# microsoft/ANCE

Measured on NVIDIA H100. Metric: ANN-refresh throughput: passages encoded/sec + queries top-200/sec, 8.8M x 768, higher is better.
Workload: dtype fp16

## Files before the change

ance_b200/csrc/attention.cuh:

```cuda
#pragma once
#include "act16.cuh"
#include "tc05.cuh"

namespace attn {

using namespace tc05;

constexpr int kTile = 128;
constexpr int kDh = 64;

__device__ __forceinline__ float ex2_ftz(float x) {
  float r;
  asm("ex2.approx.ftz.f32 %0, %1;" : "=f"(r) : "f"(x));
  return r;
}

struct Params {
  int n_tokens;
  int L;
  int heads;
  int hidden;
  const float* kbias;
  float scale_log2;
  const int32_t* row_lo;
  const int32_t* row_hi;
  const int2* tile_kv;
};

struct Smem {
  static constexpr int kStages = 3;
  static constexpr int kTileBytes = kTile * kDh * 2;
  static constexpr int kQ = 0;
  static constexpr int kKV = kQ + kTileBytes;
  static constexpr int kP = kKV + kStages * 2 * kTileBytes;
  static constexpr int kSPitch = kTile + 4;
  static constexpr int kS = kP + kTile * kTile * 2;
  static constexpr int kBias = kS + kTile * kSPitch * 4;
  static constexpr int kBiasStride = kTile * 4 + 16;
  static constexpr int kBar = kBias + kBiasStride;
  static constexpr int kNumBars = 2 + 2 * kStages;
  static constexpr int kTotal = kBar + kNumBars * 8;
  static constexpr int kDynamic = kTotal + 1024;
  static_assert(kDynamic <= 232448, "attention smem exceeds 227 KB");
};

constexpr float kRealMax = -7000.0f;

constexpr int kThreads = 256;

template <bool kPacked, bool kSingle, uint32_t FMT>
__global__ void __launch_bounds__(kThreads, 1)
attention_kernel(const __grid_constant__ CUtensorMap tmQKV, const __grid_constant__ CUtensorMap tmCTX, const Params p) {
  extern __shared__ uint8_t smem_raw[];
  uint8_t* smem = reinterpret_cast<uint8_t*>((reinterpret_cast<uintptr_t>(smem_raw) + 1023) & ~uintptr_t(1023));
  uint64_t* bars = reinterpret_cast<uint64_t*>(smem + Smem::kBar);
  uint64_t* q_full = bars + 0;
  uint64_t* q_empty = bars + 1;
  uint64_t* kv_full = bars + 2;
  uint64_t* kv_empty = bars + 2 + Smem::kStages;

  const int warp = threadIdx.x >> 5, lane = threadIdx.x & 31;
  const int n_tiles = (p.n_tokens + kTile - 1) / kTile;
  const int total_work = n_tiles * p.heads;
  const int nkv_dense = (p.L >= kTile) ? p.L / kTile : 1;
  auto kv_of = [&](int tile, int& kv0, int& nkv) {
    if constexpr (kPacked && !kSingle) {
      const int2 t = __ldg(p.tile_kv + tile);
      kv0 = t.x;
      nkv = t.y;
    } else {
      kv0 = (p.L >= kTile) ? (tile * kTile / p.L) * p.L : tile * kTile;
      nkv = nkv_dense;
    }
  };

  if (warp == 0 && lane == 0) {
    tma_prefetch_desc(&tmQKV);
    tma_prefetch_desc(&tmCTX);
    mbar_init(q_full, 1);
    mbar_init(q_empty, 4);
    for (int s = 0; s < Smem::kStages; ++s) {
      mbar_init(&kv_full[s], 1);
      mbar_init(&kv_empty[s], 4);
    }
    fence_barrier_init();
  }
  __syncthreads();

  if (warp == 0) {
    if (lane == 0) {
      Ring<Smem::kStages> kv;
      uint32_t qc = 0;
      for (int w = blockIdx.x; w < total_work; w += gridDim.x) {
        const int tile = w / p.heads, h = w - tile * p.heads;
        const int tok0 = tile * kTile;
        int kv_tok0, nkv;
        kv_of(tile, kv_tok0, nkv);
        for (int j = 0; j < nkv; ++j) {
          if (j == 0) {
            mbar_wait(q_empty, (qc & 1) ^ 1, 10);
            ++qc;
            mbar_arrive_expect_tx(q_full, Smem::kTileBytes);
            tma_load_2d(smem + Smem::kQ, &tmQKV, q_full, h * kDh, tok0, kEvictFirst);
          }
          mbar_wait(&kv_empty[kv.stage], kv.phase ^ 1, 11);
          mbar_arrive_expect_tx(&kv_full[kv.stage], 2 * Smem::kTileBytes);
          uint8_t* st = smem + Smem::kKV + kv.stage * 2 * Smem::kTileBytes;
          tma_load_2d(st, &tmQKV, &kv_full[kv.stage], p.hidden + h * kDh, kv_tok0 + j * kTile, kEvictNormal);
          tma_load_2d(st + Smem::kTileBytes, &tmQKV, &kv_full[kv.stage], 2 * p.hidden + h * kDh, kv_tok0 + j * kTile,
                      kEvictNormal);
          kv.advance();
        }
      }
    }
  } else if (warp >= 4) {
    const int quad = warp & 3;
    const int row = quad * 32 + lane;
    uint8_t* sP = smem + Smem::kP;
    float* sS = reinterpret_cast<float*>(smem + Smem::kS);
    const uint32_t srow = smem_u32(sS) / 4u + static_cast<uint32_t>(row * Smem::kSPitch);
    float* sbias = reinterpret_cast<float*>(smem + Smem::kBias);
    unsigned* smask = reinterpret_cast<unsigned*>(sbias + kTile);
    const int bar_id = 1;
    const uint32_t sq = smem_u32(smem + Smem::kQ);
    const uint32_t sp = smem_u32(sP);
    Ring<Smem::kStages> kv;
    uint32_t qc = 0;
    auto load_bias = [&](int w2, int j2) -> float {
      if (w2 >= total_work) return 0.f;
      int k0, nk;
      kv_of(w2 / p.heads, k0, nk);
      const int kt = k0 + j2 * kTile + row;
      return (kt < p.n_tokens) ? __ldg(p.kbias + kt) : -INFINITY;
    };
    auto store_chunks = [&](uint8_t* rowp, int chunk0, const uint32_t* pk) {
#pragma unroll
      for (int q = 0; q < 4; ++q) {
        const int ch = (chunk0 + q) ^ (row & 7);
        *reinterpret_cast<uint4*>(rowp + ch * 16) = make_uint4(pk[q * 4], pk[q * 4 + 1], pk[q * 4 + 2], pk[q * 4 + 3]);
      }
    };
    float bv = load_bias(blockIdx.x, 0);
    for (int w = blockIdx.x; w < total_work; w += gridDim.x) {
      const int tile = w / p.heads, h = w - tile * p.heads;
      const int tok0 = tile * kTile;
      int kv0, nkv;
      kv_of(tile, kv0, nkv);
      const bool varlen = kPacked && p.row_lo != nullptr;
      int seq_lo = (p.L >= kTile) ? 0 : (row / p.L) * p.L;
      int seq_hi = (p.L >= kTile) ? kTile : seq_lo + p.L;
      if (varlen) {
        seq_lo = __ldg(p.row_lo + tok0 + row) - kv0;
        seq_hi = __ldg(p.row_hi + tok0 + row) - kv0;
      }
      const int seq_full = seq_lo + ((seq_hi - seq_lo) & ~31);
      float m_run = -INFINITY, l_run = 0.f;
      float o[kDh];
      if constexpr (!kSingle) {
#pragma unroll
        for (int i = 0; i < kDh; ++i) o[i] = 0.f;
      }
      for (int j = 0; j < nkv; ++j) {
        sbias[row] = bv;
        {
          const unsigned mk = __ballot_sync(0xffffffffu, bv < 0.f);
          if (lane == 0) smask[quad] = mk;
        }
        if (row == 0) bulk_wait_read_all();
        named_bar_sync(bar_id, kTile);
        bv = (j + 1 < nkv) ? load_bias(w, j + 1) : load_bias(w + gridDim.x, 0);
        const unsigned mk[4] = {smask[0], smask[1], smask[2], smask[3]};
        const int bl = seq_lo - j * kTile, bh = seq_hi - j * kTile;
        const int bf = seq_full - j * kTile;
        const bool plain = kPacked ? (varlen && bl <= 0 && bh >= kTile) : ((mk[0] | mk[1] | mk[2] | mk[3]) == 0u);
        int st[4];
        if (varlen) {
#pragma unroll
          for (int c = 0; c < 4; ++c)
            st[c] = (bh <= c * 32 || bl >= c * 32 + 32) ? 0 : (bl <= c * 32 && (kSingle ? bh : bf) >= c * 32 + 32) ? 1 : 2;
        } else {
          bool own[4], any_unmasked = false;
#pragma unroll
          for (int c = 0; c < 4; ++c) {
            own[c] = !kPacked || (p.L >= 32 ? (c * 32 >= seq_lo && c * 32 < seq_hi) : c == quad);
            any_unmasked |= own[c] && mk[c] != 0xffffffffu;
          }
          const bool skip_ok = (kPacked && p.L < 32) ? false : (any_unmasked || (!kSingle && m_run > kRealMax));
#pragma unroll
          for (int c = 0; c < 4; ++c)
            st[c] = !own[c] ? 0 : (mk[c] == 0xffffffffu && skip_ok) ? 0 : (mk[c] == 0u && !(kPacked && p.L < 32)) ? 1 : 2;
        }
        if (j == 0) mbar_wait(q_full, qc & 1, 12);
        mbar_wait(&kv_full[kv.stage], kv.phase, 13);
        const uint32_t sk = smem_u32(smem + Smem::kKV + kv.stage * 2 * Smem::kTileBytes);
        {
          float s0[kTile / 2], s1[kTile / 2];
#pragma unroll
          for (int i = 0; i < kTile / 2; ++i) s0[i] = s1[i] = 0.f;
          wgmma_fence();
#pragma unroll
          for (int k = 0; k < kDh / 16; ++k) {
            const uint64_t bdesc = make_desc_k_sw128(sk + k * 32);
            wgmma_n128<FMT, 0>(s0, make_desc_k_sw128(sq + k * 32), bdesc, 1u);
            wgmma_n128<FMT, 0>(s1, make_desc_k_sw128(sq + 64 * 128 + k * 32), bdesc, 1u);
          }
          wgmma_commit();
          wgmma_wait<0>();
          wgmma_fence_regs(s0);
          wgmma_fence_regs(s1);
          acc_store_frag(sS, Smem::kSPitch, 0, 0, s0);
          acc_store_frag(sS, Smem::kSPitch, 64, 0, s1);
        }
        if (j == nkv - 1) {
          __syncwarp();
          if (lane == 0) mbar_arrive(q_empty);
          ++qc;
        }
        named_bar_sync(bar_id, kTile);
        float rsum, alpha = 1.f, m_new;
        bool all_skip = false;
        if constexpr (kSingle) {
          uint32_t v[kTile];
#pragma unroll
          for (int c = 0; c < kTile; c += 32) acc_ld_x32(srow + c, v + c);
          float mx[4] = {-INFINITY, -INFINITY, -INFINITY, -INFINITY};
          if (plain) {
#pragma unroll
            for (int i = 0; i < kTile; ++i) mx[i & 3] = fmaxf(mx[i & 3], __uint_as_float(v[i]));
          } else {
#pragma unroll
            for (int c = 0; c < kTile; c += 32) {
              if (st[c >> 5] == 1) {
#pragma unroll
                for (int i = c; i < c + 32; ++i) {
                  const float t = __uint_as_float(v[i]) * p.scale_log2;
                  v[i] = __float_as_uint(t);
                  mx[i & 3] = fmaxf(mx[i & 3], t);
                }
              } else if (st[c >> 5] == 2) {
#pragma unroll
                for (int i = c; i < c + 32; ++i) {
                  float t = fmaf(__uint_as_float(v[i]), p.scale_log2, sbias[i]);
                  if (kPacked && (i < bl || i >= bh)) t = -INFINITY;
                  v[i] = __float_as_uint(t);
                  mx[i & 3] = fmaxf(mx[i & 3], t);
                }
              }
            }
          }
          m_new = fmaxf(fmaxf(mx[0], mx[1]), fmaxf(mx[2], mx[3]));
          const float sc = plain ? p.scale_log2 : 1.0f;
          if (plain) m_new *= p.scale_log2;
          const float nm = -m_new;
          float rs[4] = {0.f, 0.f, 0.f, 0.f};
#pragma unroll
          for (int c = 0; c < kTile; c += 32) {
            uint32_t pk[16];
            if (st[c >> 5] == 0) {
#pragma unroll
              for (int i = 0; i < 16; ++i) pk[i] = 0u;
            } else {
#pragma unroll
              for (int i = 0; i < 32; i += 2) {
                const float p0 = ex2_ftz(fmaf(__uint_as_float(v[c + i]), sc, nm));
                const float p1 = ex2_ftz(fmaf(__uint_as_float(v[c + i + 1]), sc, nm));
                rs[(i >> 1) & 3] += p0 + p1;
                pk[i >> 1] = act16::Act<FMT>::pack2(p0, p1);
              }
            }
            store_chunks(sP + (c >> 6) * (kTile * 128) + row * 128, (c & 63) >> 3, pk);
          }
          rsum = (rs[0] + rs[1]) + (rs[2] + rs[3]);
        } else {
          const int stb = st[0] | (st[1] << 2) | (st[2] << 4) | (st[3] << 6);
          all_skip = stb == 0;
          auto exp_pass = [&](float m_ref, float& rs_out) -> float {
            float rs_ = 0.f, mu = -INFINITY;
            const float nm = -m_ref;
#pragma unroll 1
            for (int c = 0; c < kTile; c += 32) {
              const int sc_ = (stb >> (c >> 4)) & 3;
              uint32_t pk[16];
              if (sc_ == 0) {
#pragma unroll
                for (int i = 0; i < 16; ++i) pk[i] = 0u;
              } else {
                uint32_t v[32];
                acc_ld_x32(srow + c, v);
                if (sc_ == 1) {
#pragma unroll
                  for (int i = 0; i < 32; i += 2) {
                    const float u0 = fmaf(__uint_as_float(v[i]), p.scale_log2, nm);
                    const float u1 = fmaf(__uint_as_float(v[i + 1]), p.scale_log2, nm);
                    mu = fmaxf(mu, fmaxf(u0, u1));
                    const float p0 = ex2_ftz(u0), p1 = ex2_ftz(u1);
                    rs_ += p0 + p1;
                    pk[i >> 1] = act16::Act<FMT>::pack2(p0, p1);
                  }
                } else {
#pragma unroll
                  for (int i = 0; i < 32; i += 2) {
                    float u0 = fmaf(__uint_as_float(v[i]), p.scale_log2, sbias[c + i]) + nm;
                    float u1 = fmaf(__uint_as_float(v[i + 1]), p.scale_log2, sbias[c + i + 1]) + nm;
                    if constexpr (kPacked) {
                      const int k0 = c + i, k1 = c + i + 1;
                      u0 = (k0 < bl || k0 >= bh) ? -INFINITY : (k0 < bf) ? fmaf(__uint_as_float(v[i]), p.scale_log2, nm) : u0;
                      u1 = (k1 < bl || k1 >= bh) ? -INFINITY : (k1 < bf) ? fmaf(__uint_as_float(v[i + 1]), p.scale_log2, nm) : u1;
                    }
                    mu = fmaxf(mu, fmaxf(u0, u1));
                    const float p0 = ex2_ftz(u0), p1 = ex2_ftz(u1);
                    rs_ += p0 + p1;
                    pk[i >> 1] = act16::Act<FMT>::pack2(p0, p1);
                  }
                }
              }
              store_chunks(sP + (c >> 6) * (kTile * 128) + row * 128, (c & 63) >> 3, pk);
            }
            rs_out = rs_;
            return mu;
          };
          const bool optimistic = __all_sync(0xffffffffu, j > 0 && m_run > kRealMax);
          if (optimistic) {
            m_new = m_run;
            alpha = 1.f;
            rsum = 0.f;
            float over = -INFINITY;
            if (!all_skip) {
              over = exp_pass(m_run, rsum);
            } else {
              float dummy;
              exp_pass(m_run, dummy);
            }
            if (__any_sync(0xffffffffu, over > 8.0f)) {
              m_new = fmaxf(m_run, m_run + over);
              alpha = exp2f(m_run - m_new);
              exp_pass(m_new, rsum);
            }
          } else {
            float m_blk = -INFINITY;
            if (!all_skip) {
#pragma unroll 1
              for (int c = 0; c < kTile; c += 32) {
                const int sc_ = (stb >> (c >> 4)) & 3;
                if (sc_ == 0) continue;
                uint32_t v[32];
                acc_ld_x32(srow + c, v);
                if (plain) {
#pragma unroll
                  for (int i = 0; i < 32; ++i) m_blk = fmaxf(m_blk, __uint_as_float(v[i]));
                } else if (sc_ == 1) {
#pragma unroll
                  for (int i = 0; i < 32; ++i) m_blk = fmaxf(m_blk, __uint_as_float(v[i]) * p.scale_log2);
                } else {
#pragma unroll
                  for (int i = 0; i < 32; ++i) {
                    float t = fmaf(__uint_as_float(v[i]), p.scale_log2, sbias[c + i]);
                    if (kPacked && (c + i < bl || c + i >= bh)) t = -INFINITY;
                    m_blk = fmaxf(m_blk, t);
                  }
                }
              }
            }
            if (plain) m_blk *= p.scale_log2;
            m_new = fmaxf(m_run, m_blk);
            alpha = (m_run == -INFINITY) ? 0.f : exp2f(m_run - m_new);
            exp_pass(m_new, rsum);
          }
        }
        fence_proxy_async_smem();
        named_bar_sync(bar_id, kTile);
        {
          const uint32_t sv = sk + Smem::kTileBytes;
          float o0[kDh / 2], o1[kDh / 2];
#pragma unroll
          for (int i = 0; i < kDh / 2; ++i) o0[i] = o1[i] = 0.f;
          wgmma_fence();
#pragma unroll
          for (int k = 0; k < kTile / 16; ++k) {
            const uint32_t pa = sp + (k >> 2) * (kTile * 128) + (k & 3) * 32;
            const uint64_t bdesc = make_desc_mn_sw128(sv + k * 2048, kTile * 128, 1024);
            wgmma_n64<FMT, 1>(o0, make_desc_k_sw128(pa), bdesc, 1u);
            wgmma_n64<FMT, 1>(o1, make_desc_k_sw128(pa + 64 * 128), bdesc, 1u);
          }
          wgmma_commit();
          wgmma_wait<0>();
          wgmma_fence_regs(o0);
          wgmma_fence_regs(o1);
          __syncwarp();
          if (lane == 0) mbar_arrive(&kv_empty[kv.stage]);
          kv.advance();
          acc_store_frag(sS, Smem::kSPitch, 0, 0, o0);
          acc_store_frag(sS, Smem::kSPitch, 64, 0, o1);
        }
        named_bar_sync(bar_id, kTile);
        if constexpr (kSingle) {
          l_run = rsum;
        } else {
          if (!all_skip) {
#pragma unroll
            for (int c = 0; c < kDh; c += 32) {
              uint32_t v[32];
              acc_ld_x32(srow + c, v);
#pragma unroll
              for (int i = 0; i < 32; ++i) o[c + i] = fmaf(o[c + i], alpha, __uint_as_float(v[i]));
            }
            l_run = fmaf(l_run, alpha, rsum);
            m_run = m_new;
          }
        }
      }
      {
        const float inv = 1.0f / l_run;
        if constexpr (kSingle) {
          uint32_t v[kDh];
          acc_ld_x32(srow, v);
          acc_ld_x32(srow + 32, v + 32);
#pragma unroll
          for (int i = 0; i < kDh; ++i) o[i] = __uint_as_float(v[i]);
        }
#pragma unroll
        for (int c = 0; c < kDh; c += 32) {
          uint32_t pk[16];
#pragma unroll
          for (int i = 0; i < 32; i += 2) {
            pk[i >> 1] = act16::Act<FMT>::pack2(o[c + i] * inv, o[c + i + 1] * inv);
          }
          store_chunks(sP + row * 128, c >> 3, pk);
        }
        fence_proxy_async_smem();
        named_bar_sync(bar_id, kTile);
        if (row == 0) {
          tma_store_2d(&tmCTX, sP, h * kDh, tok0);
          bulk_commit_group();
        }
      }
    }
    if (row == 0) bulk_wait_read_all();
  }

}

}
```

ance_b200/csrc/encoder.cu:

```cuda
#include <math.h>
#include <stdlib.h>
#include <string.h>

#include <map>
#include <vector>

#include "attention.cuh"
#include "common.h"
#include "encoder_bwd.cuh"
#include "gemm_store.cuh"

namespace {

constexpr float kLog2e = 1.4426950408889634f;

struct EmbedParams {
  const int32_t* ids;
  const int32_t* lens;
  const uint8_t* mask;
  int B, L, H;
  int roberta;
  int pad_id, vocab, max_pos;
  const float* word;
  const float* pos;
// ... 454 lines not shown
  if (C && R && !gemm::make_store_tmap(&p.tmR, const_cast<uint16_t*>(R), M, N, static_cast<int>(ldr))) {
    ance::set_error("encoder: cuTensorMapEncodeTiled failed for the residual (M=%d N=%d)", M, N);
    return ANCE_ERR_CUDA;
  }
  p.C = C;
  p.C32 = C32;
  p.bias = bias;
  p.R = R;
  p.ldc = N;
  p.ldc32 = N;
  p.ldr = static_cast<int>(ldr);
  p.act = act;
  {
    ance::ProfScope ps(cls, st);
    ANCE_CUDA((gemm::launch<Ep, BN, STAGES, CG, EW, FMT>(tmA, tmB, ws, p, 0, st)));
  }
  ance::count_launch(1);
  return ANCE_OK;
}

int g_ln_rows_per_warp = 2;

template <uint32_t FMT>
int layer_norm(const void* in, bool in_f32, size_t in_ld, int rows, int H, const float* g, const float* b, float eps,
               uint16_t* out16, float* out32, cudaStream_t st) {
  const int blocks = (rows + 7) / 8;
  const int nv = H / 256;
  ance::ProfScope ps(ance::kClsNorm, st);
  if (!in_f32 && out16 && !out32 && nv == 3 && g_ln_rows_per_warp > 1 && rows >= 4096) {
    const uint16_t* src = reinterpret_cast<const uint16_t*>(in);
    if (g_ln_rows_per_warp == 2) ln_rows_multi_kernel<3, 2, FMT><<<(rows + 15) / 16, 256, 0, st>>>(src, in_ld, rows, H, g, b, eps, out16);
    else if (g_ln_rows_per_warp == 3) ln_rows_packed_kernel<3, 2, FMT><<<(rows + 15) / 16, 256, 0, st>>>(src, in_ld, rows, H, g, b, eps, out16);
    else ln_rows_multi_kernel<3, 4, FMT><<<(rows + 31) / 32, 256, 0, st>>>(src, in_ld, rows, H, g, b, eps, out16);
    ANCE_CUDA(cudaGetLastError());
    ance::count_launch(1);
    return ANCE_OK;
  }
#define LN_CASE(NV_)                                                                                            \
  if (in_f32) ln_rows_kernel<NV_, true, FMT><<<blocks, 256, 0, st>>>(in, in_ld, rows, H, g, b, eps, out16, out32); \
  else ln_rows_kernel<NV_, false, FMT><<<blocks, 256, 0, st>>>(in, in_ld, rows, H, g, b, eps, out16, out32)
  if (nv == 3) { LN_CASE(3); }
  else if (nv == 4) { LN_CASE(4); }
  else if (nv == 1) { LN_CASE(1); }
  else if (nv == 2) { LN_CASE(2); }
  else { ance::set_error("encoder: hidden size %d unsupported", H); return ANCE_ERR_UNSUPPORTED; }
#undef LN_CASE
  ANCE_CUDA(cudaGetLastError());
  ance::count_launch(1);
  return ANCE_OK;
}

template <uint32_t FMT>
int set_attention_attrs() {
  ANCE_CUDA(cudaFuncSetAttribute(attn::attention_kernel<false, false, FMT>, cudaFuncAttributeMaxDynamicSharedMemorySize, attn::Smem::kDynamic));
  ANCE_CUDA(cudaFuncSetAttribute(attn::attention_kernel<false, true, FMT>, cudaFuncAttributeMaxDynamicSharedMemorySize, attn::Smem::kDynamic));
  ANCE_CUDA(cudaFuncSetAttribute(attn::attention_kernel<true, true, FMT>, cudaFuncAttributeMaxDynamicSharedMemorySize, attn::Smem::kDynamic));
  ANCE_CUDA(cudaFuncSetAttribute(attn::attention_kernel<true, false, FMT>, cudaFuncAttributeMaxDynamicSharedMemorySize, attn::Smem::kDynamic));
  return ANCE_OK;
}

struct AttentionLaunch {
  CUtensorMap tmQKV, tmCTX;
  attn::Params ap;
  int grid;
  bool packed, single;
};

int make_attention(AttentionLaunch& a, const uint16_t* qkv, uint16_t* ctx, int n_tokens, int L, int heads,
                   const float* kbias, const int32_t* row_lo, const int32_t* row_hi, const int2* tile_kv) {
  const int H = heads * attn::kDh;
  if (!tc05_host::make_tmap_2d_16b(&a.tmQKV, qkv, n_tokens, 3 * H, 3 * H, attn::kTile)) {
    ance::set_error("encoder: cuTensorMapEncodeTiled failed for QKV");
    return ANCE_ERR_CUDA;
  }
  if (!tc05_host::make_tmap_2d_16b(&a.tmCTX, ctx, n_tokens, H, H, attn::kTile)) {
    ance::set_error("encoder: cuTensorMapEncodeTiled failed for the attention output");
    return ANCE_ERR_CUDA;
  }
  const bool varlen = row_lo != nullptr;
  const bool varlen_long = varlen && L > attn::kTile;
  attn::Params& ap = a.ap;
  ap.n_tokens = n_tokens; ap.L = (varlen && !varlen_long) ? 64 : L; ap.heads = heads; ap.hidden = H;
  ap.kbias = kbias;
  ap.scale_log2 = kLog2e / 8.0f;
  ap.row_lo = varlen ? row_lo : nullptr;
  ap.row_hi = varlen ? row_hi : nullptr;
  ap.tile_kv = varlen ? tile_kv : nullptr;
  const int attn_work = ((n_tokens + 127) / 128) * heads;
  a.grid = std::min(attn_work, gemm::sm_count());
  a.packed = varlen || L < attn::kTile;
  a.single = !varlen_long && L <= attn::kTile;
  return ANCE_OK;
}

template <uint32_t FMT>
int run_attention(const AttentionLaunch& a, cudaStream_t st) {
  ance::prof_begin(ance::kClsAttn, st);
  if (a.packed && !a.single) attn::attention_kernel<true, false, FMT><<<a.grid, attn::kThreads, attn::Smem::kDynamic, st>>>(a.tmQKV, a.tmCTX, a.ap);
  else if (a.packed) attn::attention_kernel<true, true, FMT><<<a.grid, attn::kThreads, attn::Smem::kDynamic, st>>>(a.tmQKV, a.tmCTX, a.ap);
  else if (a.single) attn::attention_kernel<false, true, FMT><<<a.grid, attn::kThreads, attn::Smem::kDynamic, st>>>(a.tmQKV, a.tmCTX, a.ap);
  else attn::attention_kernel<false, false, FMT><<<a.grid, attn::kThreads, attn::Smem::kDynamic, st>>>(a.tmQKV, a.tmCTX, a.ap);
  ance::prof_end(ance::kClsAttn, st);
  ANCE_CUDA(cudaGetLastError());
  ance::count_launch(1);
  return ANCE_OK;
}

struct TrainLayout {
  size_t ids, kbias, layers, per_layer, x_in, qkv, ctx, t1, x1, u, ff, t2, x_final, head_in, total;
};
constexpr int kTrainLayoutFields = 15;
static_assert(sizeof(TrainLayout) == kTrainLayoutFields * sizeof(size_t), "ance_dbg_train_layout lists every field");

TrainLayout train_layout(const ance_encoder_config& c, int B, int L) {
  const size_t M = static_cast<size_t>(B) * L, H = c.hidden, F = c.ffn;
  auto up = [](size_t x) { return (x + 255) / 256 * 256; };
  TrainLayout t;
  size_t o = 0;
  t.ids = o; o += up(M * 4);
  t.kbias = o; o += up(M * 4);
  t.layers = o;
  size_t p = 0;
  t.x_in = p; p += up(M * H * 2);
  t.qkv = p; p += up(M * 3 * H * 2);
  t.ctx = p; p += up(M * H * 2);
  t.t1 = p; p += up(M * H * 2);
  t.x1 = p; p += up(M * H * 2);
  t.u = p; p += up(M * F * 2);
  t.ff = p; p += up(M * F * 2);
  t.t2 = p; p += up(M * H * 2);
  t.per_layer = p;
  o += p * c.n_layer;
  t.x_final = o; o += up(static_cast<size_t>(B) * H * 2);
  t.head_in = o; o += up(static_cast<size_t>(B) * H * 4);
  t.total = o;
  return t;
}

struct TrainSave {
  uint8_t* ws;
  TrainLayout lo;
  int n_layer;
  uint16_t* at(int l, size_t off) const { return reinterpret_cast<uint16_t*>(ws + lo.layers + l * lo.per_layer + off); }
  uint16_t* x(int l) const { return l == n_layer ? reinterpret_cast<uint16_t*>(ws + lo.x_final) : at(l, lo.x_in); }
  int32_t* ids() const { return reinterpret_cast<int32_t*>(ws + lo.ids); }
  float* kbias() const { return reinterpret_cast<float*>(ws + lo.kbias); }
  float* head_in() const { return reinterpret_cast<float*>(ws + lo.head_in); }
};

template <uint32_t FMT>
int forward_impl(ance_encoder* e, const int32_t* ids_dev, const int32_t* lens_dev, const uint8_t* mask_dev, int B, int L,
                 float* out_dev, cudaStream_t st, int n_tiles = 0, const TrainSave* ts = nullptr) {
  const ance_encoder_config& c = e->cfg;
  const bool varlen = n_tiles > 0;
// ... 1034 lines not shown
```

ance_b200/csrc/tc05.cuh:

```cuda
#pragma once

#include <cuda.h>
#include <cuda_bf16.h>
#include <cuda_fp16.h>
#include <cuda_runtime.h>
#include <stdint.h>
#include <stdio.h>

namespace tc05 {

__device__ __forceinline__ uint32_t smem_u32(const void* p) {
  return static_cast<uint32_t>(__cvta_generic_to_shared(p));
}

__device__ __forceinline__ uint32_t cluster_ctarank() {
  uint32_t r;
  asm volatile("mov.u32 %0, %%cluster_ctarank;" : "=r"(r));
  return r;
}

__device__ __forceinline__ void cluster_sync_all() {
  asm volatile("barrier.cluster.arrive.release.aligned;\n" ::: "memory");
  asm volatile("barrier.cluster.wait.acquire.aligned;\n" ::: "memory");
}
// ... 111 lines not shown
  d |= static_cast<uint64_t>((smem_addr & 0x3FFFFu) >> 4);
  d |= static_cast<uint64_t>((lbo_bytes >> 4) & 0x3FFFu) << 16;
  d |= static_cast<uint64_t>((sbo_bytes >> 4) & 0x3FFFu) << 32;
  d |= static_cast<uint64_t>(1) << 62;
  return d;
}

enum : uint32_t { kFmtF16 = 0, kFmtBF16 = 1 };

__device__ __forceinline__ void wgmma_fence() { asm volatile("wgmma.fence.sync.aligned;" ::: "memory"); }
__device__ __forceinline__ void wgmma_commit() { asm volatile("wgmma.commit_group.sync.aligned;" ::: "memory"); }
template <int N>
__device__ __forceinline__ void wgmma_wait() { asm volatile("wgmma.wait_group.sync.aligned %0;" ::"n"(N) : "memory"); }
template <int R>
__device__ __forceinline__ void wgmma_fence_regs(float (&d)[R]) {
#pragma unroll
  for (int i = 0; i < R; ++i) asm volatile("" : "+f"(d[i])::"memory");
}

#define TC05_R8(i) "+f"(d[i]), "+f"(d[i + 1]), "+f"(d[i + 2]), "+f"(d[i + 3]), "+f"(d[i + 4]), "+f"(d[i + 5]), "+f"(d[i + 6]), "+f"(d[i + 7])
#define TC05_R32 TC05_R8(0), TC05_R8(8), TC05_R8(16), TC05_R8(24)
#define TC05_R64 TC05_R32, TC05_R8(32), TC05_R8(40), TC05_R8(48), TC05_R8(56)
#define TC05_S32                                                                  \
  "%0, %1, %2, %3, %4, %5, %6, %7, %8, %9, %10, %11, %12, %13, %14, %15, "        \
  "%16, %17, %18, %19, %20, %21, %22, %23, %24, %25, %26, %27, %28, %29, %30, %31"
#define TC05_S64                                                                  \
  TC05_S32 ", "                                                                   \
  "%32, %33, %34, %35, %36, %37, %38, %39, %40, %41, %42, %43, %44, %45, %46, %47, " \
  "%48, %49, %50, %51, %52, %53, %54, %55, %56, %57, %58, %59, %60, %61, %62, %63"
#define TC05_WGMMA(NAME, INSTR, NR, SLIST, RLIST, IA, IB, IP, IT)                                                     \
  template <int kTransB>                                                                                              \
  __device__ __forceinline__ void NAME(float (&d)[NR], uint64_t adesc, uint64_t bdesc, uint32_t accumulate) {        \
    asm volatile("{\n\t.reg .pred p;\n\tsetp.ne.b32 p, %" IP ", 0;\n\t" INSTR " {" SLIST "}, %" IA ", %" IB           \
                 ", p, 1, 1, 0, %" IT ";\n\t}"                                                                        \
                 : RLIST                                                                                              \
                 : "l"(adesc), "l"(bdesc), "r"(accumulate), "n"(kTransB));                                            \
  }
TC05_WGMMA(wgmma_m64n128k16_bf16, "wgmma.mma_async.sync.aligned.m64n128k16.f32.bf16.bf16", 64, TC05_S64, TC05_R64, "64", "65", "66", "67")
TC05_WGMMA(wgmma_m64n128k16_f16, "wgmma.mma_async.sync.aligned.m64n128k16.f32.f16.f16", 64, TC05_S64, TC05_R64, "64", "65", "66", "67")
TC05_WGMMA(wgmma_m64n64k16_bf16, "wgmma.mma_async.sync.aligned.m64n64k16.f32.bf16.bf16", 32, TC05_S32, TC05_R32, "32", "33", "34", "35")
TC05_WGMMA(wgmma_m64n64k16_f16, "wgmma.mma_async.sync.aligned.m64n64k16.f32.f16.f16", 32, TC05_S32, TC05_R32, "32", "33", "34", "35")

template <uint32_t FMT, int kTransB>
__device__ __forceinline__ void wgmma_n128(float (&d)[64], uint64_t adesc, uint64_t bdesc, uint32_t accumulate) {
  if constexpr (FMT == kFmtBF16) wgmma_m64n128k16_bf16<kTransB>(d, adesc, bdesc, accumulate);
  else wgmma_m64n128k16_f16<kTransB>(d, adesc, bdesc, accumulate);
}
template <uint32_t FMT, int kTransB>
__device__ __forceinline__ void wgmma_n64(float (&d)[32], uint64_t adesc, uint64_t bdesc, uint32_t accumulate) {
  if constexpr (FMT == kFmtBF16) wgmma_m64n64k16_bf16<kTransB>(d, adesc, bdesc, accumulate);
  else wgmma_m64n64k16_f16<kTransB>(d, adesc, bdesc, accumulate);
}

template <int R>
__device__ __forceinline__ void acc_store_frag(float* tile, int pitch, int r0, int c0, const float (&d)[R]) {
  const int t = threadIdx.x & 127;
  const int r = r0 + 16 * (t >> 5) + ((t & 31) >> 2);
  const int c = c0 + 2 * (t & 3);
#pragma unroll
  for (int j = 0; j < R / 4; ++j) {
    *reinterpret_cast<float2*>(tile + r * pitch + c + 8 * j) = make_float2(d[4 * j], d[4 * j + 1]);
    *reinterpret_cast<float2*>(tile + (r + 8) * pitch + c + 8 * j) = make_float2(d[4 * j + 2], d[4 * j + 3]);
  }
}

__device__ __forceinline__ void acc_ld_x32(uint32_t waddr, uint32_t* v) {
#pragma unroll
  for (int i = 0; i < 32; i += 4)
    asm volatile("ld.shared.v4.u32 {%0, %1, %2, %3}, [%4];"
                 : "=r"(v[i]), "=r"(v[i + 1]), "=r"(v[i + 2]), "=r"(v[i + 3])
                 : "r"((waddr + i) * 4u)
                 : "memory");
}

template <int kStages>
struct Ring {
  uint32_t stage = 0, phase = 0;
  __device__ __forceinline__ void advance() {
    if (++stage == kStages) {
      stage = 0;
      phase ^= 1;
    }
  }
};

}

namespace tc05_host {

typedef CUresult (*EncodeTiledFn)(CUtensorMap*, CUtensorMapDataType, cuuint32_t, void*, const cuuint64_t*,
                                  const cuuint64_t*, const cuuint32_t*, const cuuint32_t*, CUtensorMapInterleave,
                                  CUtensorMapSwizzle, CUtensorMapL2promotion, CUtensorMapFloatOOBfill);

inline EncodeTiledFn encode_fn() {
  static EncodeTiledFn fn = nullptr;
  if (!fn) {
    void* p = nullptr;
    cudaDriverEntryPointQueryResult q;
    if (cudaGetDriverEntryPoint("cuTensorMapEncodeTiled", &p, cudaEnableDefault, &q) != cudaSuccess ||
        q != cudaDriverEntryPointSuccess)
      return nullptr;
    fn = reinterpret_cast<EncodeTiledFn>(p);
  }
  return fn;
}

// ... 16 lines not shown
```

Baseline: 17170.

## Add dedicated single-KV-tile attention kernel with register-resident softmax and RS wgmma

Splits attention into a multi-tile kernel and a new single-tile kernel used when the sequence fits in one 128-token tile. The new kernel runs 384 threads with two consumer warpgroups plus a producer. It loads Q/K/V per stage, computes softmax directly on the wgmma accumulator registers, and feeds the probabilities as register A-operands to a P·V wgmma. This drops the shared-memory round trips for S and P and the extra barriers of the old path. Grid sizing changes to roughly half the work count for the single path, and the new path adds register pressure and more complex masking code.

```diff
diff --git a/ance_b200/csrc/attention.cuh b/ance_b200/csrc/attention.cuh
--- a/ance_b200/csrc/attention.cuh
+++ b/ance_b200/csrc/attention.cuh
@@ -48,9 +48,9 @@
 
 constexpr int kThreads = 256;
 
-template <bool kPacked, bool kSingle, uint32_t FMT>
+template <bool kPacked, uint32_t FMT>
 __global__ void __launch_bounds__(kThreads, 1)
-attention_kernel(const __grid_constant__ CUtensorMap tmQKV, const __grid_constant__ CUtensorMap tmCTX, const Params p) {
+attention_multi_kernel(const __grid_constant__ CUtensorMap tmQKV, const __grid_constant__ CUtensorMap tmCTX, const Params p) {
   extern __shared__ uint8_t smem_raw[];
   uint8_t* smem = reinterpret_cast<uint8_t*>((reinterpret_cast<uintptr_t>(smem_raw) + 1023) & ~uintptr_t(1023));
   uint64_t* bars = reinterpret_cast<uint64_t*>(smem + Smem::kBar);
@@ -64,7 +64,7 @@
   const int total_work = n_tiles * p.heads;
   const int nkv_dense = (p.L >= kTile) ? p.L / kTile : 1;
   auto kv_of = [&](int tile, int& kv0, int& nkv) {
-    if constexpr (kPacked && !kSingle) {
+    if constexpr (kPacked) {
       const int2 t = __ldg(p.tile_kv + tile);
       kv0 = t.x;
       nkv = t.y;
@@ -156,10 +156,8 @@
       const int seq_full = seq_lo + ((seq_hi - seq_lo) & ~31);
       float m_run = -INFINITY, l_run = 0.f;
       float o[kDh];
-      if constexpr (!kSingle) {
-#pragma unroll
-        for (int i = 0; i < kDh; ++i) o[i] = 0.f;
-      }
+#pragma unroll
+      for (int i = 0; i < kDh; ++i) o[i] = 0.f;
       for (int j = 0; j < nkv; ++j) {
         sbias[row] = bv;
         {
@@ -177,7 +175,7 @@
         if (varlen) {
 #pragma unroll
           for (int c = 0; c < 4; ++c)
-            st[c] = (bh <= c * 32 || bl >= c * 32 + 32) ? 0 : (bl <= c * 32 && (kSingle ? bh : bf) >= c * 32 + 32) ? 1 : 2;
+            st[c] = (bh <= c * 32 || bl >= c * 32 + 32) ? 0 : (bl <= c * 32 && bf >= c * 32 + 32) ? 1 : 2;
         } else {
           bool own[4], any_unmasked = false;
 #pragma unroll
@@ -185,7 +183,7 @@
             own[c] = !kPacked || (p.L >= 32 ? (c * 32 >= seq_lo && c * 32 < seq_hi) : c == quad);
             any_unmasked |= own[c] && mk[c] != 0xffffffffu;
           }
-          const bool skip_ok = (kPacked && p.L < 32) ? false : (any_unmasked || (!kSingle && m_run > kRealMax));
+          const bool skip_ok = (kPacked && p.L < 32) ? false : (any_unmasked || m_run > kRealMax);
 #pragma unroll
           for (int c = 0; c < 4; ++c)
             st[c] = !own[c] ? 0 : (mk[c] == 0xffffffffu && skip_ok) ? 0 : (mk[c] == 0u && !(kPacked && p.L < 32)) ? 1 : 2;
@@ -218,154 +216,99 @@
         }
         named_bar_sync(bar_id, kTile);
         float rsum, alpha = 1.f, m_new;
-        bool all_skip = false;
-        if constexpr (kSingle) {
-          uint32_t v[kTile];
-#pragma unroll
-          for (int c = 0; c < kTile; c += 32) acc_ld_x32(srow + c, v + c);
-          float mx[4] = {-INFINITY, -INFINITY, -INFINITY, -INFINITY};
-          if (plain) {
-#pragma unroll
-            for (int i = 0; i < kTile; ++i) mx[i & 3] = fmaxf(mx[i & 3], __uint_as_float(v[i]));
-          } else {
-#pragma unroll
-            for (int c = 0; c < kTile; c += 32) {
-              if (st[c >> 5] == 1) {
-#pragma unroll
-                for (int i = c; i < c + 32; ++i) {
-                  const float t = __uint_as_float(v[i]) * p.scale_log2;
-                  v[i] = __float_as_uint(t);
-                  mx[i & 3] = fmaxf(mx[i & 3], t);
+        const int stb = st[0] | (st[1] << 2) | (st[2] << 4) | (st[3] << 6);
+        const bool all_skip = stb == 0;
+        auto exp_pass = [&](float m_ref, float& rs_out) -> float {
+          float rs_ = 0.f, mu = -INFINITY;
+          const float nm = -m_ref;
+#pragma unroll 1
+          for (int c = 0; c < kTile; c += 32) {
+            const int sc_ = (stb >> (c >> 4)) & 3;
+            uint32_t pk[16];
+            if (sc_ == 0) {
+#pragma unroll
+              for (int i = 0; i < 16; ++i) pk[i] = 0u;
+            } else {
+              uint32_t v[32];
+              acc_ld_x32(srow + c, v);
+              if (sc_ == 1) {
+#pragma unroll
+                for (int i = 0; i < 32; i += 2) {
+                  const float u0 = fmaf(__uint_as_float(v[i]), p.scale_log2, nm);
+                  const float u1 = fmaf(__uint_as_float(v[i + 1]), p.scale_log2, nm);
+                  mu = fmaxf(mu, fmaxf(u0, u1));
+                  const float p0 = ex2_ftz(u0), p1 = ex2_ftz(u1);
+                  rs_ += p0 + p1;
+                  pk[i >> 1] = act16::Act<FMT>::pack2(p0, p1);
                 }
-              } else if (st[c >> 5] == 2) {
-#pragma unroll
-                for (int i = c; i < c + 32; ++i) {
-                  float t = fmaf(__uint_as_float(v[i]), p.scale_log2, sbias[i]);
-                  if (kPacked && (i < bl || i >= bh)) t = -INFINITY;
-                  v[i] = __float_as_uint(t);
-                  mx[i & 3] = fmaxf(mx[i & 3], t);
+              } else {
+#pragma unroll
+                for (int i = 0; i < 32; i += 2) {
+                  float u0 = fmaf(__uint_as_float(v[i]), p.scale_log2, sbias[c + i]) + nm;
+                  float u1 = fmaf(__uint_as_float(v[i + 1]), p.scale_log2, sbias[c + i + 1]) + nm;
+                  if constexpr (kPacked) {
+                    const int k0 = c + i, k1 = c + i + 1;
+                    u0 = (k0 < bl || k0 >= bh) ? -INFINITY : (k0 < bf) ? fmaf(__uint_as_float(v[i]), p.scale_log2, nm) : u0;
+                    u1 = (k1 < bl || k1 >= bh) ? -INFINITY : (k1 < bf) ? fmaf(__uint_as_float(v[i + 1]), p.scale_log2, nm) : u1;
+                  }
+                  mu = fmaxf(mu, fmaxf(u0, u1));
+                  const float p0 = ex2_ftz(u0), p1 = ex2_ftz(u1);
+                  rs_ += p0 + p1;
+                  pk[i >> 1] = act16::Act<FMT>::pack2(p0, p1);
                 }
               }
             }
-          }
-          m_new = fmaxf(fmaxf(mx[0], mx[1]), fmaxf(mx[2], mx[3]));
-          const float sc = plain ? p.scale_log2 : 1.0f;
-          if (plain) m_new *= p.scale_log2;
-          const float nm = -m_new;
-          float rs[4] = {0.f, 0.f, 0.f, 0.f};
-#pragma unroll
-          for (int c = 0; c < kTile; c += 32) {
-            uint32_t pk[16];
-            if (st[c >> 5] == 0) {
-#pragma unroll
-              for (int i = 0; i < 16; ++i) pk[i] = 0u;
-            } else {
-#pragma unroll
-              for (int i = 0; i < 32; i += 2) {
-                const float p0 = ex2_ftz(fmaf(__uint_as_float(v[c + i]), sc, nm));
-                const float p1 = ex2_ftz(fmaf(__uint_as_float(v[c + i + 1]), sc, nm));
-                rs[(i >> 1) & 3] += p0 + p1;
-                pk[i >> 1] = act16::Act<FMT>::pack2(p0, p1);
-              }
-            }
             store_chunks(sP + (c >> 6) * (kTile * 128) + row * 128, (c & 63) >> 3, pk);
           }
-          rsum = (rs[0] + rs[1]) + (rs[2] + rs[3]);
+          rs_out = rs_;
+          return mu;
+        };
+        const bool optimistic = __all_sync(0xffffffffu, j > 0 && m_run > kRealMax);
+        if (optimistic) {
+          m_new = m_run;
+          alpha = 1.f;
+          rsum = 0.f;
+          float over = -INFINITY;
+          if (!all_skip) {
+            over = exp_pass(m_run, rsum);
+          } else {
+            float dummy;
+            exp_pass(m_run, dummy);
+          }
+          if (__any_sync(0xffffffffu, over > 8.0f)) {
+            m_new = fmaxf(m_run, m_run + over);
+            alpha = exp2f(m_run - m_new);
+            exp_pass(m_new, rsum);
+          }
         } else {
-          const int stb = st[0] | (st[1] << 2) | (st[2] << 4) | (st[3] << 6);
-          all_skip = stb == 0;
-          auto exp_pass = [&](float m_ref, float& rs_out) -> float {
-            float rs_ = 0.f, mu = -INFINITY;
-            const float nm = -m_ref;
+          float m_blk = -INFINITY;
+          if (!all_skip) {
 #pragma unroll 1
             for (int c = 0; c < kTile; c += 32) {
               const int sc_ = (stb >> (c >> 4)) & 3;
-              uint32_t pk[16];
-              if (sc_ == 0) {
-#pragma unroll
-                for (int i = 0; i < 16; ++i) pk[i] = 0u;
+              if (sc_ == 0) continue;
+              uint32_t v[32];
+              acc_ld_x32(srow + c, v);
+              if (plain) {
+#pragma unroll
+                for (int i = 0; i < 32; ++i) m_blk = fmaxf(m_blk, __uint_as_float(v[i]));
+              } else if (sc_ == 1) {
+#pragma unroll
+                for (int i = 0; i < 32; ++i) m_blk = fmaxf(m_blk, __uint_as_float(v[i]) * p.scale_log2);
               } else {
-                uint32_t v[32];
-                acc_ld_x32(srow + c, v);
-                if (sc_ == 1) {
-#pragma unroll
-                  for (int i = 0; i < 32; i += 2) {
-                    const float u0 = fmaf(__uint_as_float(v[i]), p.scale_log2, nm);
-                    const float u1 = fmaf(__uint_as_float(v[i + 1]), p.scale_log2, nm);
-                    mu = fmaxf(mu, fmaxf(u0, u1));
-                    const float p0 = ex2_ftz(u0), p1 = ex2_ftz(u1);
-                    rs_ += p0 + p1;
-                    pk[i >> 1] = act16::Act<FMT>::pack2(p0, p1);
-                  }
-                } else {
-#pragma unroll
-                  for (int i = 0; i < 32; i += 2) {
-                    float u0 = fmaf(__uint_as_float(v[i]), p.scale_log2, sbias[c + i]) + nm;
-                    float u1 = fmaf(__uint_as_float(v[i + 1]), p.scale_log2, sbias[c + i + 1]) + nm;
-                    if constexpr (kPacked) {
-                      const int k0 = c + i, k1 = c + i + 1;
-                      u0 = (k0 < bl || k0 >= bh) ? -INFINITY : (k0 < bf) ? fmaf(__uint_as_float(v[i]), p.scale_log2, nm) : u0;
-                      u1 = (k1 < bl || k1 >= bh) ? -INFINITY : (k1 < bf) ? fmaf(__uint_as_float(v[i + 1]), p.scale_log2, nm) : u1;
-                    }
-                    mu = fmaxf(mu, fmaxf(u0, u1));
-                    const float p0 = ex2_ftz(u0), p1 = ex2_ftz(u1);
-                    rs_ += p0 + p1;
-                    pk[i >> 1] = act16::Act<FMT>::pack2(p0, p1);
-                  }
-                }
-              }
-              store_chunks(sP + (c >> 6) * (kTile * 128) + row * 128, (c & 63) >> 3, pk);
-            }
-            rs_out = rs_;
-            return mu;
-          };
-          const bool optimistic = __all_sync(0xffffffffu, j > 0 && m_run > kRealMax);
-          if (optimistic) {
-            m_new = m_run;
-            alpha = 1.f;
-            rsum = 0.f;
-            float over = -INFINITY;
-            if (!all_skip) {
-              over = exp_pass(m_run, rsum);
-            } else {
-              float dummy;
-              exp_pass(m_run, dummy);
-            }
-            if (__any_sync(0xffffffffu, over > 8.0f)) {
-              m_new = fmaxf(m_run, m_run + over);
-              alpha = exp2f(m_run - m_new);
-              exp_pass(m_new, rsum);
-            }
-          } else {
-            float m_blk = -INFINITY;
-            if (!all_skip) {
-#pragma unroll 1
-              for (int c = 0; c < kTile; c += 32) {
-                const int sc_ = (stb >> (c >> 4)) & 3;
-                if (sc_ == 0) continue;
-                uint32_t v[32];
-                acc_ld_x32(srow + c, v);
-                if (plain) {
-#pragma unroll
-                  for (int i = 0; i < 32; ++i) m_blk = fmaxf(m_blk, __uint_as_float(v[i]));
-                } else if (sc_ == 1) {
-#pragma unroll
-                  for (int i = 0; i < 32; ++i) m_blk = fmaxf(m_blk, __uint_as_float(v[i]) * p.scale_log2);
-                } else {
-#pragma unroll
-                  for (int i = 0; i < 32; ++i) {
-                    float t = fmaf(__uint_as_float(v[i]), p.scale_log2, sbias[c + i]);
-                    if (kPacked && (c + i < bl || c + i >= bh)) t = -INFINITY;
-                    m_blk = fmaxf(m_blk, t);
-                  }
+#pragma unroll
+                for (int i = 0; i < 32; ++i) {
+                  float t = fmaf(__uint_as_float(v[i]), p.scale_log2, sbias[c + i]);
+                  if (kPacked && (c + i < bl || c + i >= bh)) t = -INFINITY;
+                  m_blk = fmaxf(m_blk, t);
                 }
               }
             }
-            if (plain) m_blk *= p.scale_log2;
-            m_new = fmaxf(m_run, m_blk);
-            alpha = (m_run == -INFINITY) ? 0.f : exp2f(m_run - m_new);
-            exp_pass(m_new, rsum);
-          }
+          }
+          if (plain) m_blk *= p.scale_log2;
+          m_new = fmaxf(m_run, m_blk);
+          alpha = (m_run == -INFINITY) ? 0.f : exp2f(m_run - m_new);
+          exp_pass(m_new, rsum);
         }
         fence_proxy_async_smem();
         named_bar_sync(bar_id, kTile);
@@ -393,31 +336,20 @@
           acc_store_frag(sS, Smem::kSPitch, 64, 0, o1);
         }
         named_bar_sync(bar_id, kTile);
-        if constexpr (kSingle) {
-          l_run = rsum;
-        } else {
-          if (!all_skip) {
-#pragma unroll
-            for (int c = 0; c < kDh; c += 32) {
-              uint32_t v[32];
-              acc_ld_x32(srow + c, v);
-#pragma unroll
-              for (int i = 0; i < 32; ++i) o[c + i] = fmaf(o[c + i], alpha, __uint_as_float(v[i]));
-            }
-            l_run = fmaf(l_run, alpha, rsum);
-            m_run = m_new;
-          }
+        if (!all_skip) {
+#pragma unroll
+          for (int c = 0; c < kDh; c += 32) {
+            uint32_t v[32];
+            acc_ld_x32(srow + c, v);
+#pragma unroll
+            for (int i = 0; i < 32; ++i) o[c + i] = fmaf(o[c + i], alpha, __uint_as_float(v[i]));
+          }
+          l_run = fmaf(l_run, alpha, rsum);
+          m_run = m_new;
         }
       }
       {
         const float inv = 1.0f / l_run;
-        if constexpr (kSingle) {
-          uint32_t v[kDh];
-          acc_ld_x32(srow, v);
-          acc_ld_x32(srow + 32, v + 32);
-#pragma unroll
-          for (int i = 0; i < kDh; ++i) o[i] = __uint_as_float(v[i]);
-        }
 #pragma unroll
         for (int c = 0; c < kDh; c += 32) {
           uint32_t pk[16];
@@ -440,4 +372,250 @@
 
 }
 
+struct SmemSingle {
+  static constexpr int kStages = 2;
+  static constexpr int kTileBytes = kTile * kDh * 2;
+  static constexpr int kStageBytes = 3 * kTileBytes;
+  static constexpr int kQKV = 0;
+  static constexpr int kOut = kQKV + 2 * kStages * kStageBytes;
+  static constexpr int kBias = kOut + 2 * kTileBytes;
+  static constexpr int kBiasStride = kTile * 4 + 16;
+  static constexpr int kBar = kBias + 2 * kBiasStride;
+  static constexpr int kNumBars = 2 * 2 * kStages;
+  static constexpr int kTotal = kBar + kNumBars * 8;
+  static constexpr int kDynamic = kTotal + 1024;
+  static_assert(kDynamic <= 232448, "single-block attention smem exceeds 227 KB");
+};
+
+constexpr int kSingleThreads = 384;
+
+struct RowSt {
+  int st, bl, bh;
+  bool plain;
+};
+
+template <bool kPacked, uint32_t FMT>
+__device__ __forceinline__ void softmax_pair(float (&d)[64], const RowSt& ra, const RowSt& rb, const float* sbias, int q4,
+                                             float scale_log2, uint32_t (&pk)[32], float& la, float& lb) {
+  const RowSt rs[2] = {ra, rb};
+  float mx[2] = {-INFINITY, -INFINITY};
+#pragma unroll
+  for (int j = 0; j < 16; ++j) {
+    const int c = j >> 2;
+    const float2 b2 = *reinterpret_cast<const float2*>(sbias + 8 * j + 2 * q4);
+#pragma unroll
+    for (int e = 0; e < 4; ++e) {
+      const RowSt& r = rs[e >> 1];
+      const int col = 8 * j + 2 * q4 + (e & 1);
+      const int s = (r.st >> (2 * c)) & 3;
+      const float v = d[4 * j + e];
+      float t = fmaf(v, scale_log2, (e & 1) ? b2.y : b2.x);
+      if (kPacked && (col < r.bl || col >= r.bh)) t = -INFINITY;
+      t = r.plain ? v : (s == 1) ? v * scale_log2 : t;
+      d[4 * j + e] = t;
+      if (s != 0) mx[e >> 1] = fmaxf(mx[e >> 1], t);
+    }
+  }
+  float sc[2], nm[2];
+#pragma unroll
+  for (int i = 0; i < 2; ++i) {
+    float m = mx[i];
+    m = fmaxf(m, __shfl_xor_sync(0xffffffffu, m, 1));
+    m = fmaxf(m, __shfl_xor_sync(0xffffffffu, m, 2));
+    if (rs[i].plain) m *= scale_log2;
+    sc[i] = rs[i].plain ? scale_log2 : 1.0f;
+    nm[i] = -m;
+  }
+  float acc[2] = {0.f, 0.f};
+#pragma unroll
+  for (int j = 0; j < 16; ++j) {
+    const int c = j >> 2;
+#pragma unroll
+    for (int h = 0; h < 2; ++h) {
+      const bool zero = ((rs[h].st >> (2 * c)) & 3) == 0;
+      const float p0 = zero ? 0.f : ex2_ftz(fmaf(d[4 * j + 2 * h], sc[h], nm[h]));
+      const float p1 = zero ? 0.f : ex2_ftz(fmaf(d[4 * j + 2 * h + 1], sc[h], nm[h]));
+      acc[h] += p0 + p1;
+      pk[2 * j + h] = act16::Act<FMT>::pack2(p0, p1);
+    }
+  }
+#pragma unroll
+  for (int i = 0; i < 2; ++i) {
+    acc[i] = acc[i] + __shfl_xor_sync(0xffffffffu, acc[i], 1);
+    acc[i] = acc[i] + __shfl_xor_sync(0xffffffffu, acc[i], 2);
+  }
+  la = acc[0];
+  lb = acc[1];
 }
+
+template <bool kPacked, uint32_t FMT>
+__global__ void __launch_bounds__(kSingleThreads, 1)
+attention_single_kernel(const __grid_constant__ CUtensorMap tmQKV, const __grid_constant__ CUtensorMap tmCTX, const Params p) {
+  using S = SmemSingle;
+  extern __shared__ uint8_t smem_raw[];
+  uint8_t* smem = reinterpret_cast<uint8_t*>((reinterpret_cast<uintptr_t>(smem_raw) + 1023) & ~uintptr_t(1023));
+  uint64_t* bars = reinterpret_cast<uint64_t*>(smem + S::kBar);
+
+  const int wg = __shfl_sync(0xffffffffu, static_cast<int>(threadIdx.x >> 7), 0);
+  const int n_tiles = (p.n_tokens + kTile - 1) / kTile;
+  const int total_work = n_tiles * p.heads;
+  const int stride = 2 * gridDim.x;
+
+  if (threadIdx.x == 0) {
+    tma_prefetch_desc(&tmQKV);
+    tma_prefetch_desc(&tmCTX);
+    for (int g = 0; g < 2; ++g) {
+      for (int s = 0; s < S::kStages; ++s) {
+        mbar_init(bars + 2 * S::kStages * g + s, 1);
+        mbar_init(bars + 2 * S::kStages * g + S::kStages + s, 4);
+      }
+    }
+    fence_barrier_init();
+  }
+  __syncthreads();
+
+  if (wg == 0) {
+    const int warp = threadIdx.x >> 5, lane = threadIdx.x & 31;
+    if (warp < 2 && lane == 0) {
+      uint64_t* full = bars + 2 * S::kStages * warp;
+      uint64_t* empty = full + S::kStages;
+      uint8_t* ring = smem + S::kQKV + warp * S::kStages * S::kStageBytes;
+      Ring<S::kStages> rq;
+      for (int w = 2 * blockIdx.x + warp; w < total_work; w += stride) {
+        const int tile = w / p.heads, h = w - tile * p.heads;
+        const int tok0 = tile * kTile;
+        mbar_wait(&empty[rq.stage], rq.phase ^ 1, 20);
+        mbar_arrive_expect_tx(&full[rq.stage], S::kStageBytes);
+        uint8_t* st = ring + rq.stage * S::kStageBytes;
+        tma_load_2d(st, &tmQKV, &full[rq.stage], h * kDh, tok0, kEvictFirst);
+        tma_load_2d(st + S::kTileBytes, &tmQKV, &full[rq.stage], p.hidden + h * kDh, tok0, kEvictFirst);
+        tma_load_2d(st + 2 * S::kTileBytes, &tmQKV, &full[rq.stage], 2 * p.hidden + h * kDh, tok0, kEvictFirst);
+        rq.advance();
+      }
+    }
+    return;
+  }
+
+  const int g = wg - 1;
+  const int t = threadIdx.x & 127, warp = t >> 5, lane = t & 31, q4 = lane & 3;
+  const int r0 = 16 * warp + (lane >> 2);
+  uint64_t* full = bars + 2 * S::kStages * g;
+  uint64_t* empty = full + S::kStages;
+  const uint32_t ring = smem_u32(smem + S::kQKV + g * S::kStages * S::kStageBytes);
+  uint8_t* sout = smem + S::kOut + g * S::kTileBytes;
+  float* sbias = reinterpret_cast<float*>(smem + S::kBias + g * S::kBiasStride);
+  unsigned* smask = reinterpret_cast<unsigned*>(sbias + kTile);
+  const int bar_id = 1 + g;
+  const bool varlen = kPacked && p.row_lo != nullptr;
+  Ring<S::kStages> rq;
+  auto load_bias = [&](int w2) -> float {
+    if (w2 >= total_work) return 0.f;
+    const int kt = (w2 / p.heads) * kTile + t;
+    return (kt < p.n_tokens) ? __ldg(p.kbias + kt) : -INFINITY;
+  };
+  float bv = load_bias(2 * blockIdx.x + g);
+  for (int w = 2 * blockIdx.x + g; w < total_work; w += stride) {
+    const int tile = w / p.heads, h = w - tile * p.heads;
+    const int tok0 = tile * kTile;
+    sbias[t] = bv;
+    {
+      const unsigned mk = __ballot_sync(0xffffffffu, bv < 0.f);
+      if (lane == 0) smask[warp] = mk;
+    }
+    if (t == 0) bulk_wait_read_all();
+    named_bar_sync(bar_id, kTile);
+    bv = load_bias(w + stride);
+    const unsigned mk[4] = {smask[0], smask[1], smask[2], smask[3]};
+    RowSt rs[4];
+#pragma unroll
+    for (int i = 0; i < 4; ++i) {
+      const int row = r0 + (i & 1) * 8 + (i >> 1) * 64;
+      int lo = (p.L >= kTile) ? 0 : (row / p.L) * p.L;
+      int hi = (p.L >= kTile) ? kTile : lo + p.L;
+      if (varlen) {
+        lo = __ldg(p.row_lo + tok0 + row) - tok0;
+        hi = __ldg(p.row_hi + tok0 + row) - tok0;
+      }
+      int st = 0;
+      if (varlen) {
+#pragma unroll
+        for (int c = 0; c < 4; ++c)
+          st |= ((hi <= c * 32 || lo >= c * 32 + 32) ? 0 : (lo <= c * 32 && hi >= c * 32 + 32) ? 1 : 2) << (2 * c);
+      } else {
+        bool own[4], any_unmasked = false;
+#pragma unroll
+        for (int c = 0; c < 4; ++c) {
+          own[c] = !kPacked || (p.L >= 32 ? (c * 32 >= lo && c * 32 < hi) : c == (row >> 5));
+          any_unmasked |= own[c] && mk[c] != 0xffffffffu;
+        }
+        const bool skip_ok = (kPacked && p.L < 32) ? false : any_unmasked;
+#pragma unroll
+        for (int c = 0; c < 4; ++c)
+          st |= (!own[c] ? 0 : (mk[c] == 0xffffffffu && skip_ok) ? 0 : (mk[c] == 0u && !(kPacked && p.L < 32)) ? 1 : 2)
+                << (2 * c);
+      }
+      rs[i].st = st;
+      rs[i].bl = lo;
+      rs[i].bh = hi;
+      rs[i].plain = kPacked ? (varlen && lo <= 0 && hi >= kTile) : ((mk[0] | mk[1] | mk[2] | mk[3]) == 0u);
+    }
+
+    mbar_wait(&full[rq.stage], rq.phase, 21);
+    const uint32_t sq = ring + rq.stage * S::kStageBytes, sk = sq + S::kTileBytes, sv = sq + 2 * S::kTileBytes;
+    auto half = [&](int m0, const RowSt& ra, const RowSt& rb) {
+      uint32_t pk[32];
+      float l[2];
+      {
+        float s[kTile / 2];
+#pragma unroll
+        for (int i = 0; i < kTile / 2; ++i) s[i] = 0.f;
+        wgmma_fence();
+#pragma unroll
+        for (int k = 0; k < kDh / 16; ++k)
+          wgmma_n128<FMT, 0>(s, make_desc_k_sw128(sq + m0 * 128 + k * 32), make_desc_k_sw128(sk + k * 32), 1u);
+        wgmma_commit();
+        wgmma_wait<0>();
+        wgmma_fence_regs(s);
+        softmax_pair<kPacked, FMT>(s, ra, rb, sbias, q4, p.scale_log2, pk, l[0], l[1]);
+      }
+      float o[kDh / 2];
+#pragma unroll
+      for (int i = 0; i < kDh / 2; ++i) o[i] = 0.f;
+      wgmma_fence_regs(pk);
+      wgmma_fence();
+#pragma unroll
+      for (int k = 0; k < kTile / 16; ++k) {
+        const uint32_t a[4] = {pk[4 * k], pk[4 * k + 1], pk[4 * k + 2], pk[4 * k + 3]};
+        wgmma_n64_rs<FMT>(o, a, make_desc_mn_sw128(sv + k * 2048, kTile * 128, 1024));
+      }
+      wgmma_commit();
+      wgmma_wait<0>();
+      wgmma_fence_regs(o);
+#pragma unroll
+      for (int hh = 0; hh < 2; ++hh) {
+        const int row = m0 + r0 + 8 * hh;
+        const float inv = 1.0f / l[hh];
+        uint8_t* rowp = sout + row * 128 + q4 * 4;
+#pragma unroll
+        for (int j = 0; j < kDh / 8; ++j) {
+          const int e = 4 * j + 2 * hh;
+          *reinterpret_cast<uint32_t*>(rowp + ((j ^ (row & 7)) << 4)) = act16::Act<FMT>::pack2(o[e] * inv, o[e + 1] * inv);
+        }
+      }
+    };
+    half(0, rs[0], rs[1]);
+    half(64, rs[2], rs[3]);
+    __syncwarp();
+    if (lane == 0) mbar_arrive(&empty[rq.stage]);
+    rq.advance();
+    fence_proxy_async_smem();
+    named_bar_sync(bar_id, kTile);
+    if (t == 0) {
+      tma_store_2d(&tmCTX, sout, h * kDh, tok0);
+      bulk_commit_group();
+    }
+  }
+  if (t == 0) bulk_wait_read_all();
+}
+
+}
diff --git a/ance_b200/csrc/encoder.cu b/ance_b200/csrc/encoder.cu
--- a/ance_b200/csrc/encoder.cu
+++ b/ance_b200/csrc/encoder.cu
@@ -530,10 +530,10 @@
 
 template <uint32_t FMT>
 int set_attention_attrs() {
-  ANCE_CUDA(cudaFuncSetAttribute(attn::attention_kernel<false, false, FMT>, cudaFuncAttributeMaxDynamicSharedMemorySize, attn::Smem::kDynamic));
-  ANCE_CUDA(cudaFuncSetAttribute(attn::attention_kernel<false, true, FMT>, cudaFuncAttributeMaxDynamicSharedMemorySize, attn::Smem::kDynamic));
-  ANCE_CUDA(cudaFuncSetAttribute(attn::attention_kernel<true, true, FMT>, cudaFuncAttributeMaxDynamicSharedMemorySize, attn::Smem::kDynamic));
-  ANCE_CUDA(cudaFuncSetAttribute(attn::attention_kernel<true, false, FMT>, cudaFuncAttributeMaxDynamicSharedMemorySize, attn::Smem::kDynamic));
+  ANCE_CUDA(cudaFuncSetAttribute(attn::attention_multi_kernel<false, FMT>, cudaFuncAttributeMaxDynamicSharedMemorySize, attn::Smem::kDynamic));
+  ANCE_CUDA(cudaFuncSetAttribute(attn::attention_single_kernel<false, FMT>, cudaFuncAttributeMaxDynamicSharedMemorySize, attn::SmemSingle::kDynamic));
+  ANCE_CUDA(cudaFuncSetAttribute(attn::attention_single_kernel<true, FMT>, cudaFuncAttributeMaxDynamicSharedMemorySize, attn::SmemSingle::kDynamic));
+  ANCE_CUDA(cudaFuncSetAttribute(attn::attention_multi_kernel<true, FMT>, cudaFuncAttributeMaxDynamicSharedMemorySize, attn::Smem::kDynamic));
   return ANCE_OK;
 }
 
@@ -565,19 +565,19 @@
   ap.row_hi = varlen ? row_hi : nullptr;
   ap.tile_kv = varlen ? tile_kv : nullptr;
   const int attn_work = ((n_tokens + 127) / 128) * heads;
-  a.grid = std::min(attn_work, gemm::sm_count());
   a.packed = varlen || L < attn::kTile;
   a.single = !varlen_long && L <= attn::kTile;
+  a.grid = std::min(a.single ? (attn_work + 1) / 2 : attn_work, gemm::sm_count());
   return ANCE_OK;
 }
 
 template <uint32_t FMT>
 int run_attention(const AttentionLaunch& a, cudaStream_t st) {
   ance::prof_begin(ance::kClsAttn, st);
-  if (a.packed && !a.single) attn::attention_kernel<true, false, FMT><<<a.grid, attn::kThreads, attn::Smem::kDynamic, st>>>(a.tmQKV, a.tmCTX, a.ap);
-  else if (a.packed) attn::attention_kernel<true, true, FMT><<<a.grid, attn::kThreads, attn::Smem::kDynamic, st>>>(a.tmQKV, a.tmCTX, a.ap);
-  else if (a.single) attn::attention_kernel<false, true, FMT><<<a.grid, attn::kThreads, attn::Smem::kDynamic, st>>>(a.tmQKV, a.tmCTX, a.ap);
-  else attn::attention_kernel<false, false, FMT><<<a.grid, attn::kThreads, attn::Smem::kDynamic, st>>>(a.tmQKV, a.tmCTX, a.ap);
+  if (a.single && a.packed) attn::attention_single_kernel<true, FMT><<<a.grid, attn::kSingleThreads, attn::SmemSingle::kDynamic, st>>>(a.tmQKV, a.tmCTX, a.ap);
+  else if (a.single) attn::attention_single_kernel<false, FMT><<<a.grid, attn::kSingleThreads, attn::SmemSingle::kDynamic, st>>>(a.tmQKV, a.tmCTX, a.ap);
+  else if (a.packed) attn::attention_multi_kernel<true, FMT><<<a.grid, attn::kThreads, attn::Smem::kDynamic, st>>>(a.tmQKV, a.tmCTX, a.ap);
+  else attn::attention_multi_kernel<false, FMT><<<a.grid, attn::kThreads, attn::Smem::kDynamic, st>>>(a.tmQKV, a.tmCTX, a.ap);
   ance::prof_end(ance::kClsAttn, st);
   ANCE_CUDA(cudaGetLastError());
   ance::count_launch(1);
diff --git a/ance_b200/csrc/tc05.cuh b/ance_b200/csrc/tc05.cuh
--- a/ance_b200/csrc/tc05.cuh
+++ b/ance_b200/csrc/tc05.cuh
@@ -187,6 +187,27 @@
   else wgmma_m64n64k16_f16<kTransB>(d, adesc, bdesc, accumulate);
 }
 
+#define TC05_WGMMA_RS(NAME, INSTR)                                                                                    \
+  __device__ __forceinline__ void NAME(float (&d)[32], const uint32_t (&a)[4], uint64_t bdesc) {                     \
+    asm volatile("{\n\t.reg .pred p;\n\tsetp.ne.b32 p, %37, 0;\n\t" INSTR " {" TC05_S32                              \
+                 "}, {%32, %33, %34, %35}, %36, p, 1, 1, 1;\n\t}"                                                     \
+                 : TC05_R32                                                                                           \
+                 : "r"(a[0]), "r"(a[1]), "r"(a[2]), "r"(a[3]), "l"(bdesc), "r"(1u));                                  \
+  }
+TC05_WGMMA_RS(wgmma_m64n64k16_rs_bf16, "wgmma.mma_async.sync.aligned.m64n64k16.f32.bf16.bf16")
+TC05_WGMMA_RS(wgmma_m64n64k16_rs_f16, "wgmma.mma_async.sync.aligned.m64n64k16.f32.f16.f16")
+template <uint32_t FMT>
+__device__ __forceinline__ void wgmma_n64_rs(float (&d)[32], const uint32_t (&a)[4], uint64_t bdesc) {
+  if constexpr (FMT == kFmtBF16) wgmma_m64n64k16_rs_bf16(d, a, bdesc);
+  else wgmma_m64n64k16_rs_f16(d, a, bdesc);
+}
+template <int R>
+__device__ __forceinline__ void wgmma_fence_regs(uint32_t (&a)[R]) {
+#pragma unroll
+  for (int i = 0; i < R; ++i) asm volatile("" : "+r"(a[i])::"memory");
+}
+
+
 template <int R>
 __device__ __forceinline__ void acc_store_frag(float* tile, int pitch, int r0, int c0, const float (&d)[R]) {
   const int t = threadIdx.x & 127;
```

New measurement: 17830 (median of 6 runs). 3.9% higher.
